# taha-kms/CLASSMATE-RAG

Measured on AMD Instinct MI355X. Metric: hybrid queries/sec + recall@10 vs reference, 10M×768 chunks, 1/2/4/8 GPU, higher is better.
Workload: dtype fp32-accurate E5 (K10 f16x3 MFMA) + int8/f16/f64 dense + f64 BM25

## Files before the change

classmate-rag_amd/classmate_hip/_lib.py:

```python
from __future__ import annotations

import ctypes as C
import os
from pathlib import Path

try:
    import torch
except Exception:
    torch = None

LIB_NAME = "libclassmate_hip.so"
LIB_PATH = Path(os.environ.get("CLASSMATE_HIP_LIB", Path(__file__).with_name(LIB_NAME)))

CM_OK, CM_EINVAL, CM_ENOMEM, CM_EDEVICE, CM_EZERODIV, CM_EUNSUPPORTED = 0, -1, -2, -3, -4, -5
CM_FOP_EQ, CM_FOP_NE, CM_FOP_BITS, CM_FOP_TRUE, CM_FOP_FALSE, CM_FOP_AND, CM_FOP_OR, CM_FOP_NOT = range(1, 9)
CM_FILTER_MAX_OPS, CM_FILTER_MAX_SOURCES = 64, 16
CM_DTYPE_F32, CM_DTYPE_BF16, CM_DTYPE_F16, CM_DTYPE_I32, CM_DTYPE_I64 = 0, 1, 2, 3, 4

if not LIB_PATH.exists():
    raise ImportError(
        f"{LIB_PATH} not found: build the HIP extension first "
        f"(python -c 'import __graft_entry__ as g; g.build()' or make -C classmate-rag_amd)")

lib = C.CDLL(str(LIB_PATH), mode=C.RTLD_GLOBAL)
# ... 11 lines not shown


SIGNATURES = {
    "cm_last_error": (c_char_p,),
    "cm_version": (c_int,),
    "cm_device_count": (c_int, P(c_int)),
    "cm_stream_create_cu_masked": (c_int, c_int, P(C.c_uint32), c_int, P(c_vp)),
    "cm_stream_destroy": (c_int, c_vp),
    "cm_max_topk": (c_int,),
    "cm_dense_create": (c_int, c_int, c_i32, c_i64, P(c_vp)),
    "cm_dense_destroy": (None, c_vp),
    "cm_dense_reserve": (c_int, c_vp, c_i64),
    "cm_dense_mem_stats": (c_int, c_vp, c_vp, c_vp, c_vp),
    "cm_dense_set_growth": (c_int, c_vp, c_i32),
    "cm_dense_upsert": (c_int, c_vp, c_vp, c_vp, c_i64),
    "cm_dense_upsert_dev": (c_int, c_vp, c_vp, c_i64, c_i64, c_vp),
    "cm_dense_delete": (c_int, c_vp, c_vp, c_i64),
    "cm_dense_compact": (c_int, c_vp, c_i64, c_i32, c_vp, c_vp),
    "cm_dense_truncate": (c_int, c_vp, c_i64),
    "cm_dense_reset": (c_int, c_vp),
    "cm_dense_live_count": (c_i64, c_vp),
    "cm_dense_size": (c_i64, c_vp),
    "cm_dense_dim": (c_i32, c_vp),
    "cm_dense_search": (c_int, c_vp, c_vp, c_i32, c_i32, c_vp, c_vp, c_vp, c_vp),
    "cm_dense_search_lists": (c_int, c_vp, c_vp, c_i32, c_i32, c_vp, c_i32, c_vp, c_vp, c_vp, c_vp),
    "cm_dense_search_lists_dev": (c_int, c_vp, c_vp, c_i32, c_i32, c_vp, c_i32, c_vp, c_vp, c_vp, c_vp),
    "cm_dense_search_workspace": (c_i64, c_vp, c_i32, c_i32),
    "cm_dense_search_kind": (c_i32, c_vp, c_i32, c_i32),
    "cm_dense_set_path": (c_int, c_vp, c_i32),
    "cm_dense_workspace_fallbacks": (c_i32, c_vp, c_i32, c_i32, c_vp),
    "cm_dense_last_fallbacks": (c_i32, c_vp),
    "cm_dense_workspace_wide_reranks": (c_i32, c_vp, c_i32, c_i32, c_vp),
    "cm_dense_last_wide_reranks": (c_i32, c_vp),
    "cm_dense_timing": (c_int, c_vp, c_i32),
    "cm_dense_set_seed_event": (c_int, c_vp, c_vp),
    "cm_dense_timing_drain": (c_i32, c_vp, c_vp, c_i32),
    "cm_bm25_timing": (c_int, c_vp, c_i32),
    "cm_bm25_timing_drain": (c_i32, c_vp, c_vp, c_i32),
    "cm_dense_search_dev": (c_int, c_vp, c_vp, c_i32, c_i32, c_vp, c_vp, c_vp, c_vp, c_i64, c_vp),
    "cm_shard_merge_topk_dev": (c_int, c_vp, c_i32, c_i32, c_i32, c_i32, c_vp, c_vp, c_vp, c_vp, c_vp),
    "cm_dense_search_dev_deferred": (c_int, c_vp, c_vp, c_i32, c_i32, c_vp, c_vp, c_vp, c_vp, c_i64, c_vp),
    "cm_dense_exact_fallback_dev": (c_int, c_vp, c_vp, c_i32, c_i32, c_vp, c_vp, c_vp, c_vp, c_i64, c_vp),
    "cm_dense_export": (c_int, c_vp, c_i64, c_i64, c_vp, c_vp),
    "cm_dense_gather_dev": (c_int, c_vp, c_vp, c_i64, c_vp, c_vp),
    "cm_dense_live_bits_dev": (c_vp, c_vp),
    "cm_bm25_create": (c_int, c_int, P(c_vp)),
    "cm_bm25_destroy": (None, c_vp),
    "cm_bm25_build": (c_int, c_vp, c_vp, c_vp, c_i64, c_i32, c_vp),
    "cm_bm25_build_dev": (c_int, c_vp, c_vp, c_vp, c_i64, c_i64, c_i32, c_vp),
    "cm_bm25_append": (c_int, c_vp, c_vp, c_vp, c_i64, c_i32),
    "cm_bm25_append_dev": (c_int, c_vp, c_vp, c_vp, c_i64, c_i64, c_i32, c_vp),
    "cm_bm25_remove": (c_int, c_vp, c_vp, c_i64),
    "cm_bm25_remove_dev": (c_int, c_vp, c_vp, c_vp),
    "cm_bm25_replace": (c_int, c_vp, c_vp, c_i64, c_vp, c_vp, c_i32),
    "cm_bm25_replace_dev": (c_int, c_vp, c_vp, c_i64, c_vp, c_vp, c_i64, c_i32, c_vp),
    "cm_bm25_num_docs": (c_i64, c_vp),
    "cm_bm25_num_postings": (c_i64, c_vp),
    "cm_bm25_stats": (c_int, c_vp, P(c_i64), P(c_i64), P(c_f64), P(c_f64)),
    "cm_bm25_export": (c_int, c_vp, c_vp, c_vp, c_vp, c_vp, c_vp),
    "cm_bm25_set_head_policy": (c_int, c_vp, c_f64, c_i64),
    "cm_bm25_num_head_terms": (c_i32, c_vp),
    "cm_bm25_set_path": (c_int, c_vp, c_i32),
    "cm_bm25_workspace_rescored": (c_i32, c_vp, c_i32, c_i32, c_i32, c_vp),
    "cm_bm25_last_rescored": (c_i32, c_vp),
    "cm_bm25_term_stats": (c_int, c_vp, c_vp, c_vp),
    "cm_bm25_set_stats": (c_int, c_vp, c_vp, c_i32, c_i64, c_i64, c_f64),
# ... 87 lines not shown
```

classmate-rag_amd/classmate_hip/engine.py:

```python
from __future__ import annotations

import ctypes as C
import os
from typing import Optional, Sequence

import numpy as np

from . import _lib as L

try:
    import torch
except Exception:
    torch = None


def default_device() -> int:
    env = os.environ.get("CM_DEVICE")
    if env:
        return int(env)
    if torch is not None and torch.cuda.is_available():
        return torch.cuda.current_device()
    return 0


# ... 195 lines not shown
            raise ValueError(f"filter_of entries must be in [0, {ab.shape[0]})")
        dist = np.empty((nq, k), np.float32)
        rows = np.empty((nq, k), np.int64)
        vecs = np.empty((nq, k, self.dim), np.float32) if return_vectors else None
        if nq:
            L.check(L.fn["cm_dense_search_lists"](self._h, L.ptr(qq), nq, int(k), L.ptr(ab), int(ab.shape[0]), L.ptr(fo),
                                                  L.ptr(dist), L.ptr(rows), L.ptr(vecs)), "cm_dense_search_lists")
        return (dist, rows, vecs) if return_vectors else (dist, rows)

    def export(self, row0: int = 0, n: Optional[int] = None, with_live: bool = False):
        n = self.size - row0 if n is None else int(n)
        out = np.empty((max(n, 0), self.dim), np.float32)
        live = np.zeros(max((n + 31) // 32, 1), np.uint32) if with_live else None
        L.check(L.fn["cm_dense_export"](self._h, int(row0), n, L.ptr(out), L.ptr(live)), "cm_dense_export")
        if not with_live:
            return out
        mask = np.unpackbits(live.view(np.uint8), bitorder="little")[:n].astype(bool)
        return out, mask

    PATH_AUTO, PATH_F32, PATH_COARSE, PATH_STREAM, PATH_Q8, PATH_Q8S = 0, 1, 3, 4, 5, 6

    def set_path(self, kind: int):
        L.check(L.fn["cm_dense_set_path"](self._h, int(kind)), "cm_dense_set_path")

    def search_kind(self, nq: int, k: int) -> int:
        return int(L.fn["cm_dense_search_kind"](self._h, int(nq), int(k)))

    def last_fallbacks(self) -> int:
        return int(L.fn["cm_dense_last_fallbacks"](self._h))

    def last_wide_reranks(self) -> int:
        return int(L.fn["cm_dense_last_wide_reranks"](self._h))

    def timing(self, enable: bool = True):
        L.check(L.fn["cm_dense_timing"](self._h, int(bool(enable))), "cm_dense_timing")

    def set_seed_event(self, event=None):
        self._seed_event = event
        L.check(L.fn["cm_dense_set_seed_event"](self._h, event.cuda_event if event is not None else None),
                "cm_dense_set_seed_event")

    def timing_drain(self, cap: int = 4096) -> list:
        buf = np.zeros(cap, np.float32)
        n = int(L.fn["cm_dense_timing_drain"](self._h, L.ptr(buf), int(cap)))
        if n < 0:
            raise RuntimeError(L.last_error())
        return buf[:min(n, cap)].tolist()

    def workspace_fallbacks(self, nq: int, k: int, workspace) -> int:
        return int(L.fn["cm_dense_workspace_fallbacks"](self._h, int(nq), int(k), L.ptr(workspace)))

    def workspace_wide_reranks(self, nq: int, k: int, workspace) -> int:
        return int(L.fn["cm_dense_workspace_wide_reranks"](self._h, int(nq), int(k), L.ptr(workspace)))

    def workspace_bytes(self, nq: int, k: int) -> int:
        n = int(L.fn["cm_dense_search_workspace"](self._h, int(nq), int(k)))
        if n < 0:
            raise ValueError("bad (nq, k) for dense search")
        return n

    def search_dev(self, q, k: int, allow=None, out=None, workspace=None, defer_exact: bool = False):
        nq = q.shape[0]
        dev = q.device
        wsb = self.workspace_bytes(nq, k)
        if workspace is None:
            if self._ws is None or self._ws.numel() < wsb:
                self._ws = torch.empty(wsb, dtype=torch.uint8, device=dev)
            workspace = self._ws
        if out is None:
            out = (torch.empty((nq, k), dtype=torch.float32, device=dev),
                   torch.empty((nq, k), dtype=torch.int64, device=dev))
        name = "cm_dense_search_dev_deferred" if defer_exact else "cm_dense_search_dev"
        L.check(L.fn[name](self._h, L.ptr(q), nq, int(k), L.ptr(allow), L.ptr(out[0]), L.ptr(out[1]),
                           L.ptr(workspace), int(workspace.numel()), _stream(self.device)), name)
        return out

    def exact_fallback_dev(self, q, k: int, out, workspace=None, allow=None):
        if workspace is None:
            workspace = self._ws
        L.check(L.fn["cm_dense_exact_fallback_dev"](self._h, L.ptr(q), q.shape[0], int(k), L.ptr(allow),
                                                    L.ptr(out[0]), L.ptr(out[1]), L.ptr(workspace),
                                                    int(workspace.numel()), _stream(self.device)),
                "cm_dense_exact_fallback_dev")
        return out

    def gather_dev(self, rows, out=None):
# ... 722 lines not shown
```

classmate-rag_amd/csrc/cm_dense.hip:

```cpp
#include "cm_common.h"

#include <hipcub/hipcub.hpp>

#include <algorithm>
#include <cstdlib>
#include <cstring>
#include <memory>
#include <mutex>
#include <vector>

namespace cm {

typedef float f32x4 __attribute__((ext_vector_type(4)));

constexpr int kWaves = 8;
constexpr int kThreads = kWaves * 64;
constexpr int kRowTile = 16;
constexpr int kStepRows = kRowTile * kWaves;
constexpr int kCap = kStepRows;

struct DenseLds {
  int qfrag, invq, thr, cnt, len, list, buf, total;
};

// ... 968 lines not shown
    }
  }
}

__global__ void popcount_kernel(const uint32_t *__restrict__ bits, int64_t n_words,
                                unsigned long long *__restrict__ out) {
  int64_t i = (int64_t)blockIdx.x * blockDim.x + threadIdx.x;
  unsigned long long c = 0;
  for (; i < n_words; i += (int64_t)gridDim.x * blockDim.x) c += __popc(bits[i]);
  for (int o = 32; o > 0; o >>= 1) c += __shfl_xor(c, o);
  if ((threadIdx.x & 63) == 0 && c) atomicAdd(out, c);
}

}

using namespace cm;

struct cm_dense {
  int dev = 0;
  int dim = 0;
  int ld = 0;
  int64_t rows_alloc = 0;
  int64_t size = 0;
  float *C = nullptr;
  float *invc = nullptr;
  _Float16 *Xh = nullptr;
  int64_t xh_rows = 0;
  int8_t *Xq = nullptr;
  float2 *rmeta = nullptr;
  float *rnorm = nullptr;
  int path = 0;
  int32_t last_fallbacks = -1;
  int32_t last_wide = -1;
  KernelTimer timer;
  hipEvent_t seed_event = nullptr;
  uint32_t *live = nullptr;
  hipStream_t stream = nullptr;
  int64_t mem_cur = 0, mem_peak = 0;
  int64_t staged_growths = 0;
  int32_t grow_mode = 0;
  DevBuf staging, rows_buf, allow_buf, ws, out_buf;
  std::vector<float> host_tmp;
};

namespace {

struct DenseCfg {
  int QB, CH, KMAX, n_qgroups, n_cblocks;
  int64_t rows_per_block, rows_end;
  size_t lds;
};

int pick_chunk(int ld) {
  const int KS = ld / 16;
  if (KS % 24 == 0) return 12;
  if (KS % 16 == 0) return 8;
  return 0;
}

int g_num_cus = 0;

int num_cus(int dev) {
  if (g_num_cus == 0) {
    hipDeviceProp_t p;
    if (hipGetDeviceProperties(&p, dev) == hipSuccess) g_num_cus = p.multiProcessorCount;
    if (g_num_cus <= 0) g_num_cus = 256;
// ... 362 lines not shown
  uint32_t *fb_bound;
  int32_t *wide_ctr;
  uint32_t *wide_rows;
  uint64_t *wide_keys;
  DenseWs k1;
  size_t total;
};
CoarseWs coarse_ws_layout(const cm_dense *h, const CoarseCfg &c, int nq, int k, void *base) {
  CoarseWs w{};
  char *p = reinterpret_cast<char *>(base);
  size_t off = 0;
  const int64_t nq_pad = (int64_t)c.n_pass * c.qs;
  auto take = [&](int64_t bytes) -> char * {
    char *r = p + off;
    off += round_up(std::max<int64_t>(bytes, 1), 256);
    return r;
  };
  const int cap = c.q8 ? kQCap : kCBufCap;
  if (c.q8) {
    w.qq = reinterpret_cast<int8_t *>(take(nq_pad * h->ld));
    w.qsc = reinterpret_cast<float4 *>(take(nq_pad * 16));
  }
  w.qh = reinterpret_cast<_Float16 *>(take(nq_pad * h->ld * 2));
  w.qnorm = reinterpret_cast<float *>(take(nq_pad * 16));
  w.keys = reinterpret_cast<uint64_t *>(take((int64_t)c.n_pass * c.n_wg * c.qs * cap * 8));
  if (c.q8) w.ups = reinterpret_cast<float *>(take((int64_t)c.n_pass * c.n_wg * c.qs * cap * 4));
  w.cnt = reinterpret_cast<uint32_t *>(take((int64_t)c.n_pass * c.n_wg * c.qs * 4));
  w.mins = reinterpret_cast<float *>(take((int64_t)c.n_pass * c.n_wg_sample * c.qs * 4));
  w.seed = reinterpret_cast<float *>(take(nq_pad * 4));
  w.fb_mask = reinterpret_cast<int32_t *>(take(nq_pad * 4));
  w.fb_count = reinterpret_cast<int32_t *>(take(4));
  if (c.q8) {
    w.fb_bound = reinterpret_cast<uint32_t *>(take(nq_pad * 4));
    w.wide_ctr = reinterpret_cast<int32_t *>(take(8));
    w.wide_rows = reinterpret_cast<uint32_t *>(take((int64_t)kWideSlots * kWideCap * 4));
    w.wide_keys = reinterpret_cast<uint64_t *>(take((int64_t)kWideSlots * kWideCap * 8));
  }
  const DenseCfg kc = dense_config(h, nq, k, true);
  w.k1 = dense_ws_layout(h, kc, k, p ? p + off : nullptr);
  off += w.k1.total;
  w.total = off;
  return w;
}

int set_coarse_attrs() {
  static std::once_flag once;
  static hipError_t err = hipSuccess;
  std::call_once(once, [] {
    const std::pair<const void *, int> fs[] = {
        {reinterpret_cast<const void *>(&dense_coarse_scan_kernel<12, kK1cNql, false>), K1rLds<kK1cNql>::total},
        {reinterpret_cast<const void *>(&dense_coarse_scan_kernel<12, kK1cNql, true>), K1rLds<kK1cNql>::total},
        {reinterpret_cast<const void *>(&dense_coarse_scan_kernel<6, 0, false>), K1rLds<0>::total},
        {reinterpret_cast<const void *>(&dense_coarse_scan_kernel<6, 0, true>), K1rLds<0>::total},
        {reinterpret_cast<const void *>(&dense_rerank_kernel), kGatherCap * 12},
        {reinterpret_cast<const void *>(&dense_q8_scan_kernel<>), kQLds},
        {reinterpret_cast<const void *>(&dense_q8_scan_kernel<K1Q_LDS_SHARED>), kQLdsShared},
        {reinterpret_cast<const void *>(&dense_rerank_q8_kernel), kQRerankLds}};
    for (const auto &f : fs) {
      const hipError_t e = hipFuncSetAttribute(f.first, hipFuncAttributeMaxDynamicSharedMemorySize, f.second);
      if (e != hipSuccess) err = e;
    }
  });
  CM_HIP(err);
  return CM_OK;
}

using StreamFn = void (*)(const _Float16 *, const uint32_t *, const uint32_t *, int64_t, const _Float16 *, int,
// ... 13 lines not shown
    lds = K1rLds<kK1cNql>::total;
    return minonly ? &dense_coarse_scan_kernel<12, kK1cNql, true> : &dense_coarse_scan_kernel<12, kK1cNql, false>;
  }
  lds = K1rLds<0>::total;
  return minonly ? &dense_coarse_scan_kernel<6, 0, true> : &dense_coarse_scan_kernel<6, 0, false>;
}
using Q8Fn = void (*)(const int8_t *, const float2 *, const uint32_t *, const uint32_t *, int64_t, const int8_t *,
                      const float4 *, int, const float *, int64_t, int64_t, int, uint64_t *, float *, uint32_t *);
Q8Fn q8_kernel(bool full, size_t &lds) {
  lds = full ? kQLds : kQLdsShared;
  return full ? &dense_q8_scan_kernel<> : &dense_q8_scan_kernel<K1Q_LDS_SHARED>;
}
Q8Fn q8_stream_kernel(int nq) {
  return nq > 16 ? &dense_q8_stream_kernel<2, K1QS_RING> : &dense_q8_stream_kernel<1, K1QS_RING>;
}

int launch_exact_fallback(cm_dense *h, const float *q_dev, int nq, int k, int kind, const uint32_t *allow,
                          float *dist_dev, int64_t *row_dev, void *ws, int64_t ws_bytes, hipStream_t st);
int launch_coarse(cm_dense *h, const float *q_dev, int nq, int k, int kind, const uint32_t *allow,
                  float *dist_dev, int64_t *row_dev, void *ws, int64_t ws_bytes, hipStream_t st,
                  bool run_exact = true) {
  int rc;
  if ((rc = set_coarse_attrs())) return rc;
  const CoarseCfg c = coarse_config(h, nq, kind);
  const CoarseWs w = coarse_ws_layout(h, c, nq, k, ws);
  if ((int64_t)w.total > ws_bytes || !ws) CM_FAIL(CM_EINVAL, "dense workspace too small");
  const int64_t n_words = ceil_div(h->size, 32);
  size_t lds = 0;
  hipLaunchKernelGGL(dense_prep_planes, dim3(c.n_pass * c.qs), dim3(256), 0, st, q_dev, nq, h->dim, h->ld, w.qh,
                     w.qnorm);
  CM_HIP(hipGetLastError());
  CM_HIP(hipMemsetAsync(w.fb_count, 0, 4, st));
  if (c.q8) {
    CM_HIP(hipMemsetAsync(w.wide_ctr, 0, 8, st));
    hipLaunchKernelGGL(dense_prep_q8, dim3(c.n_pass * c.qs), dim3(256), 0, st, q_dev, nq, h->dim, h->ld, w.qq, w.qsc,
                       reinterpret_cast<const uint32_t *>(h->rnorm));
    CM_HIP(hipGetLastError());
  }
  if (c.stream) {
    hipLaunchKernelGGL(stream_kernel(h->ld, nq, true), dim3((unsigned)ceil_div(c.n_wg_sample, 4)), dim3(256), 0, st,
                       h->Xh, h->live, allow, n_words, w.qh, nq, (const float *)nullptr, c.rows_per_wg_sample,
                       c.rows_end_sample, c.n_wg_sample, c.qs, (uint64_t *)nullptr, (uint32_t *)nullptr, w.mins);
  } else {
    const CoarseFn fn = coarse_kernel(h->ld, true, lds);
    hipLaunchKernelGGL(fn, dim3((unsigned)((int64_t)c.n_pass * c.n_wg_sample)), dim3(256), lds, st, h->Xh, h->live,
                       allow, n_words, w.qh, nq, (const float *)nullptr, c.rows_per_wg_sample, c.rows_end_sample,
                       c.n_wg_sample, (uint64_t *)nullptr, (uint32_t *)nullptr, w.mins);
  }
  CM_HIP(hipGetLastError());
  hipLaunchKernelGGL(dense_seed_kernel, dim3(nq), dim3(256), 0, st, w.mins, c.n_wg_sample, c.qs, k, nq, w.qnorm,
                     h->rnorm, h->dim, w.seed, c.q8 ? 1 : 2);
  CM_HIP(hipGetLastError());
  if (kind == CM_DENSE_Q8 && h->seed_event) CM_HIP(hipEventRecord(h->seed_event, st));
  h->timer.begin(st);
  if (c.q8s) {
    hipLaunchKernelGGL(q8_stream_kernel(nq), dim3((unsigned)ceil_div(c.n_wg, 4)), dim3(256), 0, st, h->Xq, h->rmeta,
                       h->live, allow, n_words, w.qq, w.qsc, nq, (const float *)w.seed, c.rows_per_wg, c.rows_end,
                       c.n_wg, w.keys, w.ups, w.cnt);
  } else if (c.q8) {
    const Q8Fn fn = q8_kernel(run_exact || !env_knob("CM_K1Q_SHARED_LDS", true), lds);
    hipLaunchKernelGGL(fn, dim3(c.n_pass * c.n_wg), dim3(256), lds, st, h->Xq, h->rmeta, h->live, allow, n_words,
                       w.qq, w.qsc, nq, (const float *)w.seed, c.rows_per_wg, c.rows_end, c.n_wg, w.keys, w.ups, w.cnt);
  } else if (c.stream) {
    hipLaunchKernelGGL(stream_kernel(h->ld, nq, false), dim3((unsigned)ceil_div(c.n_wg, 4)), dim3(256), 0, st, h->Xh,
                       h->live, allow, n_words, w.qh, nq, (const float *)w.seed, c.rows_per_wg, c.rows_end, c.n_wg,
                       c.qs, w.keys, w.cnt, (float *)nullptr);
  } else {
    const CoarseFn fn = coarse_kernel(h->ld, false, lds);
    hipLaunchKernelGGL(fn, dim3((unsigned)((int64_t)c.n_pass * c.n_wg)), dim3(256), lds, st, h->Xh, h->live, allow,
                       n_words, w.qh, nq, (const float *)w.seed, c.rows_per_wg, c.rows_end, c.n_wg, w.keys, w.cnt,
                       (float *)nullptr);
  }
  h->timer.end(st);
  CM_HIP(hipGetLastError());
  if (c.q8) {
    hipLaunchKernelGGL(dense_rerank_q8_kernel, dim3(nq), dim3(kQRT), kQRerankLds, st, w.keys, w.ups, w.cnt, c.n_wg,
                       c.qs, k, nq, h->C, h->ld, h->dim, q_dev, w.qsc, xh_full(h) ? h->Xh : nullptr, w.qh, w.qnorm,
                       h->rnorm, dist_dev, row_dev, w.fb_mask, w.fb_count, w.fb_bound);
    CM_HIP(hipGetLastError());
    if (env_knob("CM_K1Q_WIDE", true))
      hipLaunchKernelGGL(dense_rerank_wide_kernel, dim3(nq), dim3(kWideThreads), 0, st, w.keys, w.cnt, c.n_wg, c.qs,
                         k, nq, h->C, h->ld, h->dim, q_dev, w.qsc, xh_full(h) ? h->Xh : nullptr, w.qh, w.qnorm,
                         h->rnorm, h->Xq, h->rmeta, w.qq, h->live, allow, n_words, c.rows_per_wg, c.rows_end, dist_dev,
                         row_dev, w.fb_mask, w.fb_count, w.fb_bound, w.wide_ctr, w.wide_rows, w.wide_keys);
  } else {
    hipLaunchKernelGGL(dense_rerank_kernel, dim3(nq), dim3(256), kGatherCap * 12, st, w.keys, w.cnt, c.n_wg, c.qs, k,
                       nq, h->C, h->ld, h->dim, q_dev, w.qnorm, h->rnorm, dist_dev, row_dev, w.fb_mask, w.fb_count);
  }
  CM_HIP(hipGetLastError());
  return run_exact ? launch_exact_fallback(h, q_dev, nq, k, kind, allow, dist_dev, row_dev, ws, ws_bytes, st) : CM_OK;
}

int launch_exact_fallback(cm_dense *h, const float *q_dev, int nq, int k, int kind, const uint32_t *allow,
                          float *dist_dev, int64_t *row_dev, void *ws, int64_t ws_bytes, hipStream_t st) {
  const CoarseCfg c = coarse_config(h, nq, kind);
  const CoarseWs w = coarse_ws_layout(h, c, nq, k, ws);
  if ((int64_t)w.total > ws_bytes || !ws) CM_FAIL(CM_EINVAL, "dense workspace too small");
  const DenseCfg kc = dense_config(h, nq, k, true);
  if (kc.lds > 163840) CM_FAIL(CM_EUNSUPPORTED, "dim/k too large for the LDS-resident query tile");
  hipLaunchKernelGGL(dense_prep_queries, dim3(kc.n_qgroups * kc.QB), dim3(256), 0, st, q_dev, nq, h->dim, h->ld,
                     w.k1.qp, w.k1.invq);
  CM_HIP(hipGetLastError());
  int rc;
  if ((rc = launch_dense(kc, h, allow, w.k1.qp, w.k1.invq, nq, k, w.fb_mask, w.fb_count, w.k1.cand, st))) return rc;
  hipLaunchKernelGGL(dense_merge_kernel, dim3(nq), dim3(256), 0, st, w.k1.cand, kc.n_cblocks, kc.QB, k, nq,
                     (const int32_t *)w.fb_mask, dist_dev, row_dev);
  CM_HIP(hipGetLastError());
  return CM_OK;
}

int dense_search_full(cm_dense *h, const float *q, int nq, int k, const uint32_t *allow_bits, float *out_dist,
// ... 21 lines not shown
  std::vector<uint64_t> top((size_t)kk);
  std::vector<float> qpad((size_t)h->ld, 0.f);
  for (int i = 0; i < nq; ++i) {
    double qn = 0.0;
    for (int c = 0; c < h->dim; ++c) {
      qpad[c] = q[(int64_t)i * h->dim + c];
      qn += (double)qpad[c] * qpad[c];
    }
    CM_HIP(hipMemcpyAsync(qp, qpad.data(), (size_t)h->ld * 4, hipMemcpyHostToDevice, h->stream));
    hipLaunchKernelGGL(dense_all_keys_kernel, dim3((unsigned)ceil_div(n, 16)), dim3(256), 0, h->stream, h->C, h->ld,
                       h->live, allow_dev, h->size, qp, std::sqrt(qn), keys);
    CM_HIP(hipGetLastError());
    CM_HIP(hipcub::DeviceRadixSort::SortKeys(base, tmp_bytes, keys, sorted, (int)n, 0, 64, h->stream));
    CM_HIP(hipMemcpyAsync(top.data(), sorted, (size_t)kk * 8, hipMemcpyDeviceToHost, h->stream));
    CM_HIP(hipStreamSynchronize(h->stream));
    for (int j = 0; j < k; ++j) {
      const uint64_t key = j < kk ? top[j] : kEmptyKey;
      out_dist[(int64_t)i * k + j] = key == kEmptyKey ? 0.f : f32_unorder((uint32_t)(key >> 32));
      out_row[(int64_t)i * k + j] = key == kEmptyKey ? -1 : (int64_t)(uint32_t)key;
    }
  }
  if (out_vec) {
    const size_t nr = (size_t)nq * k;
    if ((rc = h->rows_buf.ensure(nr * 8)) || (rc = h->out_buf.ensure(nr * h->dim * 4))) return rc;
    CM_HIP(hipMemcpyAsync(h->rows_buf.ptr, out_row, nr * 8, hipMemcpyHostToDevice, h->stream));
    hipLaunchKernelGGL(dense_gather_kernel, dim3((unsigned)nr), dim3(256), 0, h->stream, h->C, h->ld, h->dim,
                       h->rows_buf.as<int64_t>(), (int64_t)nr, h->size, h->out_buf.as<float>());
    CM_HIP(hipGetLastError());
    CM_HIP(hipMemcpyAsync(out_vec, h->out_buf.ptr, nr * h->dim * 4, hipMemcpyDeviceToHost, h->stream));
    CM_HIP(hipStreamSynchronize(h->stream));
  }
  h->last_fallbacks = 0;
  h->last_wide = 0;
  return CM_OK;
}

}

extern "C" {

int cm_max_topk(void) { return kMaxTopK; }

int cm_dense_create(int device, int32_t dim, int64_t capacity, cm_dense **out) {
  if (!out) CM_FAIL(CM_EINVAL, "out is NULL");
  *out = nullptr;
  if (dim <= 0 || dim > 2048) CM_FAIL(CM_EINVAL, "dim must be in [1, 2048]");
  if (capacity < 0) CM_FAIL(CM_EINVAL, "capacity must be >= 0");
  DeviceGuard dg(device);
  if (!dg.ok) CM_FAIL(CM_EDEVICE, "cannot select device " + std::to_string(device));
  cm_dense *h = new cm_dense();
  h->dev = device;
  h->dim = dim;
  int ld = (int)round_up(dim, 128);
  while (!pick_chunk(ld)) ld += 128;
  h->ld = ld;
  if (hipStreamCreateWithFlags(&h->stream, hipStreamDefault) != hipSuccess) {
    delete h;
    CM_FAIL(CM_EDEVICE, "hipStreamCreate failed");
  }
  if (hipMalloc(&h->rnorm, 16) != hipSuccess || hipMemset(h->rnorm, 0, 16) != hipSuccess) {
    cm_dense_destroy(h);
    CM_FAIL(CM_ENOMEM, "dense: out of device memory");
  }
  int rc = dense_grow(h, std::max<int64_t>(capacity, kStepRows));
  if (rc) {
    cm_dense_destroy(h);
// ... 168 lines not shown
int cm_dense_set_path(cm_dense *h, int32_t kind) {
  if (!h) CM_FAIL(CM_EINVAL, "null handle");
  if (kind < 0 || kind > CM_DENSE_Q8S) CM_FAIL(CM_EINVAL, "unknown dense path");
  h->path = kind;
  return CM_OK;
}

int32_t cm_dense_workspace_fallbacks(cm_dense *h, int32_t nq, int32_t k, const void *workspace_dev) {
  if (!h || !workspace_dev || nq <= 0 || k <= 0 || k > kMaxTopK) return -1;
  const int kind = dense_kind(h, nq, k);
  if (kind == CM_DENSE_F32) return 0;
  DeviceGuard dg(h->dev);
  const CoarseWs w = coarse_ws_layout(h, coarse_config(h, nq, kind), nq, k,
                                      const_cast<void *>(workspace_dev));
  int32_t c = -1;
  if (hipMemcpy(&c, w.fb_count, 4, hipMemcpyDeviceToHost) != hipSuccess) return -1;
  return c;
}

int32_t cm_dense_last_fallbacks(cm_dense *h) { return h ? h->last_fallbacks : -1; }

int32_t cm_dense_workspace_wide_reranks(cm_dense *h, int32_t nq, int32_t k, const void *workspace_dev) {
  if (!h || !workspace_dev || nq <= 0 || k <= 0 || k > kMaxTopK) return -1;
  const int kind = dense_kind(h, nq, k);
  if (kind != CM_DENSE_Q8 && kind != CM_DENSE_Q8S) return 0;
  DeviceGuard dg(h->dev);
  const CoarseWs w = coarse_ws_layout(h, coarse_config(h, nq, kind), nq, k, const_cast<void *>(workspace_dev));
  int32_t c[2] = {-1, -1};
  if (hipMemcpy(c, w.wide_ctr, 8, hipMemcpyDeviceToHost) != hipSuccess) return -1;
  return c[1];
}

int32_t cm_dense_last_wide_reranks(cm_dense *h) { return h ? h->last_wide : -1; }

int cm_dense_set_seed_event(cm_dense *h, void *event) {
  if (!h) CM_FAIL(CM_EINVAL, "null handle");
  h->seed_event = (hipEvent_t)event;
  return CM_OK;
}

int cm_dense_timing(cm_dense *h, int32_t enable) {
  if (!h) CM_FAIL(CM_EINVAL, "null handle");
  DeviceGuard dg(h->dev);
  h->timer.on = enable != 0;
  h->timer.used = 0;
  return CM_OK;
}

int32_t cm_dense_timing_drain(cm_dense *h, float *ms_out, int32_t cap) {
  if (!h) CM_FAIL(CM_EINVAL, "null handle");
  DeviceGuard dg(h->dev);
  const int n = h->timer.drain(ms_out, cap);
  if (n < 0) CM_FAIL(CM_EDEVICE, "event query failed");
  return n;
}

int32_t cm_dense_search_kind(cm_dense *h, int32_t nq, int32_t k) {
  if (!h || nq <= 0 || k <= 0 || k > kMaxTopK) return -1;
  return dense_kind(h, nq, k);
}

int cm_dense_search_dev(cm_dense *h, const float *q_dev, int32_t nq, int32_t k, const uint32_t *allow_dev,
                        float *dist_dev, int64_t *row_dev, void *workspace_dev, int64_t workspace_bytes,
                        void *stream) {
  if (!h) CM_FAIL(CM_EINVAL, "null handle");
  if (nq <= 0) return CM_OK;
// ... 91 lines not shown
  DeviceGuard dg(h->dev);
  if (k > kMaxTopK) return dense_search_full(h, q, nq, k, allow_bits, out_dist, out_row, out_vec);
  const int64_t wsb = cm_dense_search_workspace(h, nq, k);
  int rc;
  if ((rc = h->ws.ensure((size_t)wsb))) return rc;
  const size_t qbytes = (size_t)nq * h->dim * 4;
  const size_t obytes = (size_t)nq * k * (4 + 8);
  const size_t vbytes = out_vec ? (size_t)nq * k * h->dim * 4 : 0;
  if ((rc = h->staging.ensure(qbytes))) return rc;
  if ((rc = h->out_buf.ensure(round_up(obytes, 256) + vbytes))) return rc;
  const uint32_t *allow_dev = nullptr;
  if (allow_bits) {
    const int64_t nw = ceil_div(h->size, 32);
    if ((rc = h->allow_buf.ensure((size_t)std::max<int64_t>(nw, 1) * 4))) return rc;
    CM_HIP(hipMemcpyAsync(h->allow_buf.ptr, allow_bits, (size_t)nw * 4, hipMemcpyDefault, h->stream));
    allow_dev = h->allow_buf.as<uint32_t>();
  }
  CM_HIP(hipMemcpyAsync(h->staging.ptr, q, qbytes, hipMemcpyHostToDevice, h->stream));
  float *d_dist = h->out_buf.as<float>();
  int64_t *d_row = reinterpret_cast<int64_t *>(h->out_buf.as<char>() + round_up((int64_t)nq * k * 4, 8));
  rc = cm_dense_search_dev(h, h->staging.as<float>(), nq, k, allow_dev, d_dist, d_row, h->ws.ptr, wsb, h->stream);
  if (rc) return rc;
  float *d_vec = nullptr;
  if (out_vec) {
    d_vec = reinterpret_cast<float *>(h->out_buf.as<char>() + round_up(obytes, 256));
    rc = cm_dense_gather_dev(h, d_row, (int64_t)nq * k, d_vec, h->stream);
    if (rc) return rc;
  }
  CM_HIP(hipMemcpyAsync(out_dist, d_dist, (size_t)nq * k * 4, hipMemcpyDeviceToHost, h->stream));
  CM_HIP(hipMemcpyAsync(out_row, d_row, (size_t)nq * k * 8, hipMemcpyDeviceToHost, h->stream));
  if (out_vec) CM_HIP(hipMemcpyAsync(out_vec, d_vec, vbytes, hipMemcpyDeviceToHost, h->stream));
  h->last_fallbacks = 0;
  h->last_wide = 0;
  const int kind = dense_kind(h, nq, k);
  if (kind != CM_DENSE_F32) {
    const CoarseWs w = coarse_ws_layout(h, coarse_config(h, nq, kind), nq, k, h->ws.ptr);
    CM_HIP(hipMemcpyAsync(&h->last_fallbacks, w.fb_count, 4, hipMemcpyDeviceToHost, h->stream));
    if (w.wide_ctr) CM_HIP(hipMemcpyAsync(&h->last_wide, w.wide_ctr + 1, 4, hipMemcpyDeviceToHost, h->stream));
  }
  CM_HIP(hipStreamSynchronize(h->stream));
  return CM_OK;
}

}

#include "cm_dense_compact.inc"
#include "cm_dense_lists.inc"
```

classmate-rag_amd/csrc/cm_dense_q8.inc:

```

#ifndef K1Q_RING
#define K1Q_RING 12
#endif
#ifndef K1Q_DBG
#define K1Q_DBG 0
#endif
constexpr int kQDbg = K1Q_DBG;
constexpr int kQRing = K1Q_RING;
constexpr int kQCap = 128;
#ifndef K1Q_RR
#define K1Q_RR 4096
#endif
#ifndef K1Q_RT
#define K1Q_RT 1024
#endif
constexpr int kQBand = K1Q_RR;
constexpr int kQBand2 = K1Q_RR / 2;
constexpr int kQRT = K1Q_RT, kQRW = K1Q_RT / 64;
constexpr int kQSel = 256;
constexpr int kQMeta = 4;
#ifndef K1Q_LDS
#define K1Q_LDS (160 * 1024)
#endif
#ifndef K1Q_LDS_SHARED
// ... 660 lines not shown
      uint32_t incl = sum;
#pragma unroll
      for (int o = 1; o < 64; o <<= 1) {
        const uint32_t v = __shfl_up(incl, o);
        if (l >= o) incl += v;
      }
      const uint32_t rem = s_rem, excl = incl - sum;
      if (excl <= rem && rem < incl) {
        uint32_t r = rem - excl, b = 4u * l;
        if (r >= h0) {
          r -= h0;
          ++b;
          if (r >= h1) {
            r -= h1;
            ++b;
            if (r >= h2) {
              r -= h2;
              ++b;
            }
          }
        }
        s_prefix = prefix | (b << shift);
        s_rem = r;
      }
    }
    __syncthreads();
  }
  return s_prefix;
}

constexpr int kQGather = K1Q_RR;
constexpr int kQRows = 8;
constexpr int kQRerankLds = kQGather * 12;
__global__ void __launch_bounds__(kQRT) dense_rerank_q8_kernel(
    const uint64_t *__restrict__ keys, const float *__restrict__ ups, const uint32_t *__restrict__ cnts, int n_wg,
    int qs, int k, int nq, const float *__restrict__ C, int ld, int dim, const float *__restrict__ q,
    const float4 *__restrict__ qsc, const _Float16 *__restrict__ Xh, const _Float16 *__restrict__ Qh,
    const float *__restrict__ qnorm, const float *__restrict__ row_norms, float *__restrict__ out_dist,
    int64_t *__restrict__ out_row, int32_t *__restrict__ fb_mask, int32_t *__restrict__ fb_count,
    uint32_t *__restrict__ fb_bound) {
  const int qi = blockIdx.x;
  if (qi >= nq) return;
  const int tid = threadIdx.x, lane = tid & 63, wave = tid >> 6;
  const int qp = qi / qs, ql = qi - qp * qs;
  extern __shared__ __attribute__((aligned(16))) unsigned char dyn[];
  uint64_t *g_key = reinterpret_cast<uint64_t *>(dyn);
  uint32_t *g_up = reinterpret_cast<uint32_t *>(dyn + kQGather * 8);
  __shared__ uint32_t s_off[2049];
  __shared__ uint32_t hist[256];
  __shared__ float s_q[768];
  __shared__ int s_flag, s_total, s_band;
  __shared__ uint64_t s_sel[kQSel];
  __shared__ int s_nsel;
  static_assert(kQBand * 4 <= kQGather * 4 && kQBand * 4 <= kQGather * 4 && kQBand2 * 8 <= kQGather * 4, "K1q re-rank LDS");
  uint32_t *s_rows = g_up;
  uint64_t *s_ex = g_key;
  if (tid == 0) {
    s_flag = 0;
    s_band = 0;
    s_nsel = 0;
  }
  __syncthreads();
  if (wave == 0) {
    uint32_t run = 0;
    for (int b0 = 0; b0 < n_wg; b0 += 64) {
      const int b = b0 + lane;
      uint32_t c = b < n_wg ? cnts[((int64_t)qp * n_wg + b) * qs + ql] : 0u;
      if (c > (uint32_t)kQCap) {
        s_flag = 1;
        c = kQCap;
      }
      uint32_t incl = c;
      for (int o = 1; o < 64; o <<= 1) {
// ... 12 lines not shown
  const int total = s_total;
  auto slot_of = [&](int jj) -> int64_t {
    int lo = 0, hi = n_wg - 1;
    while (lo < hi) {
      const int mid = (lo + hi + 1) >> 1;
      if (s_off[mid] <= (uint32_t)jj) lo = mid;
      else hi = mid - 1;
    }
    return (((int64_t)qp * n_wg + lo) * qs + ql) * kQCap + (jj - s_off[lo]);
  };
  const bool gathered = total <= kQGather;
  if (gathered) {
#pragma unroll 4
    for (int jj = tid; jj < total; jj += kQRT) {
      const int64_t sl = slot_of(jj);
      g_key[jj] = keys[sl];
      g_up[jj] = f32_order(ups[sl]);
    }
  }
  for (int i = tid; i < 768; i += kQRT) s_q[i] = i < dim ? q[(int64_t)qi * dim + i] : 0.f;
  __syncthreads();
  auto key_at = [&](int jj) -> uint64_t { return gathered ? g_key[jj] : keys[slot_of(jj)]; };
  auto up_at = [&](int jj) -> uint32_t { return gathered ? g_up[jj] : f32_order(ups[slot_of(jj)]); };
  uint32_t tkey = 0xffffffffu;
  if (total >= k) tkey = block_select_fn(up_at, total, k - 1, hist);
  if (s_flag) {
    if (tid == 0) {
      fb_mask[qi] = 2;
      fb_bound[qi] = tkey;
      atomicAdd(fb_count, 1);
    }
    return;
  }
  for (int jj = tid; jj < total; jj += kQRT) {
    const uint64_t key = key_at(jj);
    if (tkey == 0xffffffffu || (uint32_t)(key >> 32) <= tkey) {
      const int p = atomicAdd(&s_band, 1);
      if (p < kQBand) s_rows[p] = (uint32_t)key;
    }
  }
  __syncthreads();
  const int band = s_band;
  if (band > kQBand) {
    if (tid == 0) {
      fb_mask[qi] = 2;
      fb_bound[qi] = tkey;
      atomicAdd(fb_count, 1);
    }
    return;
  }
  if (tid == 0) {
    fb_mask[qi] = 0;
    fb_bound[qi] = 0u;
  }
  const uint32_t *band_rows = s_rows;
  int band2 = band;
  if (Xh != nullptr) {
  float *s_dh = reinterpret_cast<float *>(dyn);
  uint32_t *s_rows2 = reinterpret_cast<uint32_t *>(dyn + kQGather * 4);
  const float Eh = coarse_err(qnorm, qi, row_norms, dim);
  {
    typedef _Float16 h2 __attribute__((ext_vector_type(2)));
    const int hl = lane & 31, hh = lane >> 5;
    f16x8 qv[3];
    int kof[3];
#pragma unroll
    for (int u = 0; u < 3; ++u) {
      const int pc = hl + 32 * u;
      kof[u] = 64 * (pc >> 3) + 32 * ((pc >> 2) & 1) + 8 * (pc & 3);
      qv[u] = *reinterpret_cast<const f16x8 *>(Qh + (int64_t)qi * ld + kof[u]);
    }
    constexpr int RP = 4;
    for (int c0 = wave * 2 * RP; c0 < band; c0 += kQRW * 2 * RP) {
      f16x8 xv[RP][3];
#pragma unroll
      for (int rp = 0; rp < RP; ++rp) {
        const int c = min(c0 + 2 * rp + hh, band - 1);
        const int64_t row = s_rows[c];
        const int64_t tile = row >> 6;
        const int rr = (int)(row & 63), rt = rr >> 4, jj = rr & 15;
// ... 4 lines not shown
              Xh + ((((tile * (ld >> 6) + cch) * 8 + rt * 2 + sb) << 9) + ((jj * 4 + gg) << 3)));
        }
      }
#pragma unroll
      for (int rp = 0; rp < RP; ++rp) {
        float acc = 0.f;
#pragma unroll
        for (int u = 0; u < 3; ++u)
#pragma unroll
          for (int e = 0; e < 8; e += 2)
            acc = __builtin_amdgcn_fdot2(h2{xv[rp][u][e], xv[rp][u][e + 1]}, h2{qv[u][e], qv[u][e + 1]}, acc, false);
#pragma unroll
        for (int o = 16; o > 0; o >>= 1) acc += __shfl_xor(acc, o);
        const int c = c0 + 2 * rp + hh;
        if (hl == 0 && c < band) s_dh[c] = 1.0f - acc;
      }
    }
  }
  __syncthreads();
  {
    const uint32_t kth_h = band >= k ? block_select_fn([&](int i) { return f32_order(s_dh[i] + Eh); }, band, k - 1, hist)
                                     : 0xffffffffu;
    if (tid == 0) s_band = 0;
    __syncthreads();
    for (int c = tid; c < band; c += kQRT)
      if (kth_h == 0xffffffffu || f32_order(s_dh[c] - Eh) <= kth_h) s_rows2[atomicAdd(&s_band, 1)] = s_rows[c];
    __syncthreads();
  }
  band2 = s_band;
  band_rows = s_rows2;
  if (band2 > kQBand2) {
    if (tid == 0) {
      fb_mask[qi] = 2;
      fb_bound[qi] = tkey;
      atomicAdd(fb_count, 1);
    }
    return;
  }
  }
  const double qnrm = (double)qsc[qi].w;
  constexpr int M = 12;
  for (int c0 = wave * kQRows; c0 < band2; c0 += kQRW * kQRows) {
    float x[kQRows][M];
    uint32_t rows[kQRows];
#pragma unroll
    for (int r = 0; r < kQRows; ++r) {
      const int c = min(c0 + r, band2 - 1);
      rows[r] = band_rows[c];
      const float *cr = C + (int64_t)rows[r] * ld + lane;
#pragma unroll
      for (int m = 0; m < M; ++m) x[r][m] = cr[64 * m];
    }
    double dq[kQRows], dc[kQRows];
#pragma unroll
    for (int r = 0; r < kQRows; ++r) {
      dq[r] = 0.0;
      dc[r] = 0.0;
#pragma unroll
      for (int m = 0; m < M; ++m) {
        const double xv = (double)x[r][m];
        dq[r] += xv * (double)s_q[lane + 64 * m];
        dc[r] += xv * xv;
      }
    }
    for (int o = 32; o > 0; o >>= 1) {
#pragma unroll
      for (int r = 0; r < kQRows; ++r) {
        dq[r] += __shfl_xor(dq[r], o);
        dc[r] += __shfl_xor(dc[r], o);
      }
    }
    if (lane == 0) {
#pragma unroll
      for (int r = 0; r < kQRows; ++r)
        if (c0 + r < band2) {
          const float dist = (float)(1.0 - dq[r] / ((sqrt(dc[r]) + 1e-30) * (qnrm + 1e-30)));
          s_ex[c0 + r] = ((uint64_t)f32_order(dist) << 32) | rows[r];
        }
    }
  }
  __syncthreads();
  const uint32_t thi = band2 > k ? block_select_fn([&](int i) { return (uint32_t)(s_ex[i] >> 32); }, band2, k - 1, hist)
                                : 0xffffffffu;
  for (int c = tid; c < band2; c += kQRT) {
    const uint64_t key = s_ex[c];
    if ((uint32_t)(key >> 32) <= thi) {
      const int p = atomicAdd(&s_nsel, 1);
      if (p < kQSel) s_sel[p] = key;
    }
  }
  __syncthreads();
  const int nsel = s_nsel;
  const uint64_t *cand = nsel <= kQSel ? s_sel : s_ex;
  const int ncand = nsel <= kQSel ? nsel : band2;
  for (int c = tid; c < ncand; c += kQRT) {
    const uint64_t key = cand[c];
    int rank = 0;
    for (int i = 0; i < ncand; ++i) rank += cand[i] < key ? 1 : 0;
    if (rank < k) {
      out_dist[(int64_t)qi * k + rank] = f32_unorder((uint32_t)(key >> 32));
      out_row[(int64_t)qi * k + rank] = (int64_t)(uint32_t)key;
    }
  }
  for (int i = band2 + tid; i < k; i += kQRT) {
    out_dist[(int64_t)qi * k + i] = 0.f;
    out_row[(int64_t)qi * k + i] = -1;
  }
}

constexpr int kWideSlots = 16;
constexpr int kWideCap = 1 << 16;
constexpr int kWideThreads = 1024;
constexpr int kWideOvf = 64;
// ... 235 lines not shown
```

include/classmate_hip.h:

```cpp
#ifndef CLASSMATE_HIP_H
#define CLASSMATE_HIP_H

#include <stddef.h>
#include <stdint.h>

#ifdef __cplusplus
extern "C" {
#endif

#define CM_OK 0
#define CM_EINVAL (-1)
#define CM_ENOMEM (-2)
#define CM_EDEVICE (-3)
#define CM_EZERODIV (-4)
#define CM_EUNSUPPORTED (-5)

#define CM_DTYPE_F32 0
#define CM_DTYPE_BF16 1
#define CM_DTYPE_F16 2
#define CM_DTYPE_I32 3
#define CM_DTYPE_I64 4

const char *cm_last_error(void);
int cm_version(void);
// ... 9 lines not shown
int cm_dense_reserve(cm_dense *h, int64_t capacity);
int cm_dense_mem_stats(cm_dense *h, int64_t *cur_bytes, int64_t *peak_bytes, int64_t *staged_growths);
int cm_dense_set_growth(cm_dense *h, int32_t mode);
int cm_dense_upsert(cm_dense *h, const float *vecs, const int64_t *rows, int64_t n);
int cm_dense_upsert_dev(cm_dense *h, const float *vecs_dev, int64_t row0, int64_t n, void *stream);
int cm_dense_delete(cm_dense *h, const int64_t *rows, int64_t n);
int cm_dense_compact(cm_dense *h, int64_t expect_live, int32_t shrink, int64_t *old_rows_out, int64_t *new_size);
int cm_dense_truncate(cm_dense *h, int64_t new_size);
int cm_dense_reset(cm_dense *h);
int64_t cm_dense_live_count(cm_dense *h);
int64_t cm_dense_size(cm_dense *h);
int32_t cm_dense_dim(cm_dense *h);
int cm_dense_search(cm_dense *h, const float *q, int32_t nq, int32_t k, const uint32_t *allow_bits,
                    float *out_dist, int64_t *out_row, float *out_vec);
int cm_dense_search_lists(cm_dense *h, const float *q, int32_t nq, int32_t k, const uint32_t *allow_bits,
                          int32_t n_filters, const int32_t *filter_of, float *out_dist, int64_t *out_row,
                          float *out_vec);
int cm_dense_search_lists_dev(cm_dense *h, const float *q_dev, int32_t nq, int32_t k, const uint32_t *allow_bits,
                              int32_t n_filters, const int32_t *filter_of, float *dist_dev, int64_t *row_dev,
                              void *stream);
int64_t cm_dense_search_workspace(cm_dense *h, int32_t nq, int32_t k);
#define CM_DENSE_F32 1
#define CM_DENSE_F16X3 2
#define CM_DENSE_COARSE 3
#define CM_DENSE_STREAM 4
#define CM_DENSE_Q8 5
#define CM_DENSE_Q8S 6
int32_t cm_dense_search_kind(cm_dense *h, int32_t nq, int32_t k);
int cm_dense_set_path(cm_dense *h, int32_t kind);
int32_t cm_dense_workspace_fallbacks(cm_dense *h, int32_t nq, int32_t k, const void *workspace_dev);
int32_t cm_dense_last_fallbacks(cm_dense *h);
int32_t cm_dense_workspace_wide_reranks(cm_dense *h, int32_t nq, int32_t k, const void *workspace_dev);
int32_t cm_dense_last_wide_reranks(cm_dense *h);
int cm_dense_timing(cm_dense *h, int32_t enable);
int cm_dense_set_seed_event(cm_dense *h, void *event);
int32_t cm_dense_timing_drain(cm_dense *h, float *ms_out, int32_t cap);
int cm_dense_search_dev(cm_dense *h, const float *q_dev, int32_t nq, int32_t k, const uint32_t *allow_dev,
                        float *dist_dev, int64_t *row_dev, void *workspace_dev, int64_t workspace_bytes,
                        void *stream);
int cm_dense_search_dev_deferred(cm_dense *h, const float *q_dev, int32_t nq, int32_t k, const uint32_t *allow_dev,
                                 float *dist_dev, int64_t *row_dev, void *workspace_dev, int64_t workspace_bytes,
                                 void *stream);
int cm_dense_exact_fallback_dev(cm_dense *h, const float *q_dev, int32_t nq, int32_t k, const uint32_t *allow_dev,
                                float *dist_dev, int64_t *row_dev, void *workspace_dev, int64_t workspace_bytes,
                                void *stream);
int cm_dense_export(cm_dense *h, int64_t row0, int64_t n, float *out, uint32_t *live_out);
int cm_dense_gather_dev(cm_dense *h, const int64_t *rows_dev, int64_t n, float *out_dev, void *stream);
const uint32_t *cm_dense_live_bits_dev(cm_dense *h);

typedef struct cm_bm25 cm_bm25;

int cm_bm25_create(int device, cm_bm25 **out);
void cm_bm25_destroy(cm_bm25 *h);
int cm_bm25_build(cm_bm25 *h, const int32_t *term_ids, const int64_t *doc_off, int64_t ndocs, int32_t vocab,
                  const uint8_t *live);
int cm_bm25_build_dev(cm_bm25 *h, const int32_t *term_ids_dev, const int64_t *doc_off_dev, int64_t ndocs,
                      int64_t ntokens, int32_t vocab, void *stream);
int cm_bm25_append(cm_bm25 *h, const int32_t *term_ids, const int64_t *doc_off, int64_t n_new, int32_t vocab);
int cm_bm25_append_dev(cm_bm25 *h, const int32_t *term_ids_dev, const int64_t *doc_off_dev, int64_t n_new,
                       int64_t ntokens, int32_t vocab, void *stream);
int cm_bm25_remove(cm_bm25 *h, const int64_t *rows, int64_t n_rows);
int cm_bm25_remove_dev(cm_bm25 *h, const uint32_t *remove_bits_dev, void *stream);
int cm_bm25_replace(cm_bm25 *h, const int64_t *rows, int64_t n_rows, const int32_t *term_ids, const int64_t *doc_off,
                    int32_t vocab);
int cm_bm25_replace_dev(cm_bm25 *h, const int64_t *rows_dev, int64_t n_rows, const int32_t *term_ids_dev,
                        const int64_t *doc_off_dev, int64_t ntokens, int32_t vocab, void *stream);
// ... 132 lines not shown
```

Before: 34640.

## Add pilot exact-rerank to tighten q8 band bound before full rerank

In the q8 rerank kernel, candidates whose upper bound is at or below the top-k threshold are first scored exactly in fp64 as a pilot set. Their k-th exact distance, plus a small pad, gives a tighter bound that shrinks the band of rows needing exact reranking and may avoid overflow fallbacks. The exact-scoring loop is factored into a templated helper, and a device counter of band rows is added for diagnostics. It adds extra block syncs and a selection pass per query, and correctness depends on the padded pilot bound staying conservative.

After: 35110 (median of 6 runs). 1.01x the previous value.

```diff
diff --git a/classmate-rag_amd/classmate_hip/_lib.py b/classmate-rag_amd/classmate_hip/_lib.py
--- a/classmate-rag_amd/classmate_hip/_lib.py
+++ b/classmate-rag_amd/classmate_hip/_lib.py
@@ -67,6 +67,8 @@
     "cm_dense_last_fallbacks": (c_i32, c_vp),
     "cm_dense_workspace_wide_reranks": (c_i32, c_vp, c_i32, c_i32, c_vp),
     "cm_dense_last_wide_reranks": (c_i32, c_vp),
+    "cm_dense_workspace_band_rows": (c_i64, c_vp, c_i32, c_i32, c_vp),
+    "cm_dense_last_band_rows": (c_i64, c_vp),
     "cm_dense_timing": (c_int, c_vp, c_i32),
     "cm_dense_set_seed_event": (c_int, c_vp, c_vp),
     "cm_dense_timing_drain": (c_i32, c_vp, c_vp, c_i32),
diff --git a/classmate-rag_amd/classmate_hip/engine.py b/classmate-rag_amd/classmate_hip/engine.py
--- a/classmate-rag_amd/classmate_hip/engine.py
+++ b/classmate-rag_amd/classmate_hip/engine.py
@@ -251,6 +251,9 @@
     def last_wide_reranks(self) -> int:
         return int(L.fn["cm_dense_last_wide_reranks"](self._h))
 
+    def last_band_rows(self) -> int:
+        return int(L.fn["cm_dense_last_band_rows"](self._h))
+
     def timing(self, enable: bool = True):
         L.check(L.fn["cm_dense_timing"](self._h, int(bool(enable))), "cm_dense_timing")
 
@@ -271,6 +274,9 @@
 
     def workspace_wide_reranks(self, nq: int, k: int, workspace) -> int:
         return int(L.fn["cm_dense_workspace_wide_reranks"](self._h, int(nq), int(k), L.ptr(workspace)))
+
+    def workspace_band_rows(self, nq: int, k: int, workspace) -> int:
+        return int(L.fn["cm_dense_workspace_band_rows"](self._h, int(nq), int(k), L.ptr(workspace)))
 
     def workspace_bytes(self, nq: int, k: int) -> int:
         n = int(L.fn["cm_dense_search_workspace"](self._h, int(nq), int(k)))
diff --git a/classmate-rag_amd/csrc/cm_dense.hip b/classmate-rag_amd/csrc/cm_dense.hip
--- a/classmate-rag_amd/csrc/cm_dense.hip
+++ b/classmate-rag_amd/csrc/cm_dense.hip
@@ -1024,6 +1024,7 @@
   int path = 0;
   int32_t last_fallbacks = -1;
   int32_t last_wide = -1;
+  int64_t last_band = -1;
   KernelTimer timer;
   hipEvent_t seed_event = nullptr;
   uint32_t *live = nullptr;
@@ -1452,7 +1453,7 @@
   w.fb_count = reinterpret_cast<int32_t *>(take(4));
   if (c.q8) {
     w.fb_bound = reinterpret_cast<uint32_t *>(take(nq_pad * 4));
-    w.wide_ctr = reinterpret_cast<int32_t *>(take(8));
+    w.wide_ctr = reinterpret_cast<int32_t *>(take(16));
     w.wide_rows = reinterpret_cast<uint32_t *>(take((int64_t)kWideSlots * kWideCap * 4));
     w.wide_keys = reinterpret_cast<uint64_t *>(take((int64_t)kWideSlots * kWideCap * 8));
   }
@@ -1532,7 +1533,7 @@
   CM_HIP(hipGetLastError());
   CM_HIP(hipMemsetAsync(w.fb_count, 0, 4, st));
   if (c.q8) {
-    CM_HIP(hipMemsetAsync(w.wide_ctr, 0, 8, st));
+    CM_HIP(hipMemsetAsync(w.wide_ctr, 0, 16, st));
     hipLaunchKernelGGL(dense_prep_q8, dim3(c.n_pass * c.qs), dim3(256), 0, st, q_dev, nq, h->dim, h->ld, w.qq, w.qsc,
                        reinterpret_cast<const uint32_t *>(h->rnorm));
     CM_HIP(hipGetLastError());
@@ -1574,9 +1575,11 @@
   h->timer.end(st);
   CM_HIP(hipGetLastError());
   if (c.q8) {
+    const bool pilot = env_knob("CM_K1Q_PILOT", true);
     hipLaunchKernelGGL(dense_rerank_q8_kernel, dim3(nq), dim3(kQRT), kQRerankLds, st, w.keys, w.ups, w.cnt, c.n_wg,
                        c.qs, k, nq, h->C, h->ld, h->dim, q_dev, w.qsc, xh_full(h) ? h->Xh : nullptr, w.qh, w.qnorm,
-                       h->rnorm, dist_dev, row_dev, w.fb_mask, w.fb_count, w.fb_bound);
+                       h->rnorm, dist_dev, row_dev, w.fb_mask, w.fb_count, w.fb_bound,
+                       pilot ? 1 : 0, reinterpret_cast<unsigned long long *>(w.wide_ctr + 2));
     CM_HIP(hipGetLastError());
     if (env_knob("CM_K1Q_WIDE", true))
       hipLaunchKernelGGL(dense_rerank_wide_kernel, dim3(nq), dim3(kWideThreads), 0, st, w.keys, w.cnt, c.n_wg, c.qs,
@@ -1664,6 +1667,7 @@
   }
   h->last_fallbacks = 0;
   h->last_wide = 0;
+  h->last_band = 0;
   return CM_OK;
 }
 
@@ -1898,6 +1902,19 @@
 }
 
 int32_t cm_dense_last_wide_reranks(cm_dense *h) { return h ? h->last_wide : -1; }
+
+int64_t cm_dense_workspace_band_rows(cm_dense *h, int32_t nq, int32_t k, const void *workspace_dev) {
+  if (!h || !workspace_dev || nq <= 0 || k <= 0 || k > kMaxTopK) return -1;
+  const int kind = dense_kind(h, nq, k);
+  if (kind != CM_DENSE_Q8 && kind != CM_DENSE_Q8S) return 0;
+  DeviceGuard dg(h->dev);
+  const CoarseWs w = coarse_ws_layout(h, coarse_config(h, nq, kind), nq, k, const_cast<void *>(workspace_dev));
+  int64_t c = -1;
+  if (hipMemcpy(&c, w.wide_ctr + 2, 8, hipMemcpyDeviceToHost) != hipSuccess) return -1;
+  return c;
+}
+
+int64_t cm_dense_last_band_rows(cm_dense *h) { return h ? h->last_band : -1; }
 
 int cm_dense_set_seed_event(cm_dense *h, void *event) {
   if (!h) CM_FAIL(CM_EINVAL, "null handle");
@@ -2055,11 +2072,15 @@
   if (out_vec) CM_HIP(hipMemcpyAsync(out_vec, d_vec, vbytes, hipMemcpyDeviceToHost, h->stream));
   h->last_fallbacks = 0;
   h->last_wide = 0;
+  h->last_band = 0;
   const int kind = dense_kind(h, nq, k);
   if (kind != CM_DENSE_F32) {
     const CoarseWs w = coarse_ws_layout(h, coarse_config(h, nq, kind), nq, k, h->ws.ptr);
     CM_HIP(hipMemcpyAsync(&h->last_fallbacks, w.fb_count, 4, hipMemcpyDeviceToHost, h->stream));
-    if (w.wide_ctr) CM_HIP(hipMemcpyAsync(&h->last_wide, w.wide_ctr + 1, 4, hipMemcpyDeviceToHost, h->stream));
+    if (w.wide_ctr) {
+      CM_HIP(hipMemcpyAsync(&h->last_wide, w.wide_ctr + 1, 4, hipMemcpyDeviceToHost, h->stream));
+      CM_HIP(hipMemcpyAsync(&h->last_band, w.wide_ctr + 2, 8, hipMemcpyDeviceToHost, h->stream));
+    }
   }
   CM_HIP(hipStreamSynchronize(h->stream));
   return CM_OK;
diff --git a/classmate-rag_amd/csrc/cm_dense_q8.inc b/classmate-rag_amd/csrc/cm_dense_q8.inc
--- a/classmate-rag_amd/csrc/cm_dense_q8.inc
+++ b/classmate-rag_amd/csrc/cm_dense_q8.inc
@@ -716,13 +716,59 @@
 constexpr int kQGather = K1Q_RR;
 constexpr int kQRows = 8;
 constexpr int kQRerankLds = kQGather * 12;
+constexpr uint32_t kQPilotPad = 4;
+constexpr int kQPilotRows = 2;
+constexpr uint64_t kQTaken = ~0ull;
+
+template <int NR, typename R>
+__device__ __forceinline__ void q8_exact_rows(const R *src, int n, int c0, int stride, const float *__restrict__ C,
+                                              int ld, const float *s_q, double qnrm, int lane, uint64_t *out) {
+  constexpr int M = 12;
+  float x[NR][M];
+  uint32_t rows[NR];
+#pragma unroll
+  for (int r = 0; r < NR; ++r) {
+    rows[r] = (uint32_t)src[min(c0 + r * stride, n - 1)];
+    const float *cr = C + (int64_t)rows[r] * ld + lane;
+#pragma unroll
+    for (int m = 0; m < M; ++m) x[r][m] = cr[64 * m];
+  }
+  double dq[NR], dc[NR];
+#pragma unroll
+  for (int r = 0; r < NR; ++r) {
+    dq[r] = 0.0;
+    dc[r] = 0.0;
+#pragma unroll
+    for (int m = 0; m < M; ++m) {
+      const double xv = (double)x[r][m];
+      dq[r] += xv * (double)s_q[lane + 64 * m];
+      dc[r] += xv * xv;
+    }
+  }
+  for (int o = 32; o > 0; o >>= 1) {
+#pragma unroll
+    for (int r = 0; r < NR; ++r) {
+      dq[r] += __shfl_xor(dq[r], o);
+      dc[r] += __shfl_xor(dc[r], o);
+    }
+  }
+  if (lane == 0) {
+#pragma unroll
+    for (int r = 0; r < NR; ++r)
+      if (c0 + r * stride < n) {
+        const float dist = (float)(1.0 - dq[r] / ((sqrt(dc[r]) + 1e-30) * (qnrm + 1e-30)));
+        out[c0 + r * stride] = ((uint64_t)f32_order(dist) << 32) | rows[r];
+      }
+  }
+}
+
 __global__ void __launch_bounds__(kQRT) dense_rerank_q8_kernel(
     const uint64_t *__restrict__ keys, const float *__restrict__ ups, const uint32_t *__restrict__ cnts, int n_wg,
     int qs, int k, int nq, const float *__restrict__ C, int ld, int dim, const float *__restrict__ q,
     const float4 *__restrict__ qsc, const _Float16 *__restrict__ Xh, const _Float16 *__restrict__ Qh,
     const float *__restrict__ qnorm, const float *__restrict__ row_norms, float *__restrict__ out_dist,
     int64_t *__restrict__ out_row, int32_t *__restrict__ fb_mask, int32_t *__restrict__ fb_count,
-    uint32_t *__restrict__ fb_bound) {
+    uint32_t *__restrict__ fb_bound, int pilot, unsigned long long *__restrict__ band_ctr) {
   const int qi = blockIdx.x;
   if (qi >= nq) return;
   const int tid = threadIdx.x, lane = tid & 63, wave = tid >> 6;
@@ -801,20 +847,54 @@
     }
     return;
   }
+  const double qnrm = (double)qsc[qi].w;
+  uint32_t bound = tkey;
+  int npilot = 0;
+  if (pilot && Xh == nullptr && total >= k) {
+    for (int jj = tid; jj < total; jj += kQRT) {
+      if (up_at(jj) <= tkey) {
+        const int p = atomicAdd(&s_nsel, 1);
+        if (p < kQSel) s_sel[p] = (uint64_t)jj;
+      }
+    }
+    __syncthreads();
+    npilot = s_nsel;
+    __syncthreads();
+    if (tid == 0) s_nsel = 0;
+    if (npilot <= kQSel) {
+      static_assert(kQSel <= kQRT, "one thread per pilot row");
+      if (tid < npilot) {
+        const int jj = (int)s_sel[tid];
+        s_sel[tid] = (uint32_t)key_at(jj);
+        if (gathered) g_key[jj] = kQTaken;
+      }
+      __syncthreads();
+      for (int c0 = wave; c0 < npilot; c0 += kQRW * kQPilotRows)
+        q8_exact_rows<kQPilotRows>(s_sel, npilot, c0, kQRW, C, ld, s_q, qnrm, lane, s_sel);
+      __syncthreads();
+      const uint32_t pkey = block_select_fn([&](int i) { return (uint32_t)(s_sel[i] >> 32); }, npilot, k - 1, hist);
+      bound = min(tkey, pkey <= 0xffffffffu - kQPilotPad ? pkey + kQPilotPad : 0xffffffffu);
+    } else {
+      npilot = 0;
+    }
+  }
+  const bool pilot_by_up = npilot > 0 && !gathered;
   for (int jj = tid; jj < total; jj += kQRT) {
     const uint64_t key = key_at(jj);
-    if (tkey == 0xffffffffu || (uint32_t)(key >> 32) <= tkey) {
+    if (key == kQTaken || (pilot_by_up && up_at(jj) <= tkey)) continue;
+    if (bound == 0xffffffffu || (uint32_t)(key >> 32) <= bound) {
       const int p = atomicAdd(&s_band, 1);
       if (p < kQBand) s_rows[p] = (uint32_t)key;
     }
   }
   __syncthreads();
   const int band = s_band;
-  if (band > kQBand) {
+  if (band + npilot > kQBand) {
     if (tid == 0) {
       fb_mask[qi] = 2;
-      fb_bound[qi] = tkey;
+      fb_bound[qi] = bound;
       atomicAdd(fb_count, 1);
+      if (npilot) atomicAdd(band_ctr, (unsigned long long)npilot);
     }
     return;
   }
@@ -885,53 +965,17 @@
   if (band2 > kQBand2) {
     if (tid == 0) {
       fb_mask[qi] = 2;
-      fb_bound[qi] = tkey;
+      fb_bound[qi] = bound;
       atomicAdd(fb_count, 1);
     }
     return;
   }
   }
-  const double qnrm = (double)qsc[qi].w;
-  constexpr int M = 12;
-  for (int c0 = wave * kQRows; c0 < band2; c0 += kQRW * kQRows) {
-    float x[kQRows][M];
-    uint32_t rows[kQRows];
-#pragma unroll
-    for (int r = 0; r < kQRows; ++r) {
-      const int c = min(c0 + r, band2 - 1);
-      rows[r] = band_rows[c];
-      const float *cr = C + (int64_t)rows[r] * ld + lane;
-#pragma unroll
-      for (int m = 0; m < M; ++m) x[r][m] = cr[64 * m];
-    }
-    double dq[kQRows], dc[kQRows];
-#pragma unroll
-    for (int r = 0; r < kQRows; ++r) {
-      dq[r] = 0.0;
-      dc[r] = 0.0;
-#pragma unroll
-      for (int m = 0; m < M; ++m) {
-        const double xv = (double)x[r][m];
-        dq[r] += xv * (double)s_q[lane + 64 * m];
-        dc[r] += xv * xv;
-      }
-    }
-    for (int o = 32; o > 0; o >>= 1) {
-#pragma unroll
-      for (int r = 0; r < kQRows; ++r) {
-        dq[r] += __shfl_xor(dq[r], o);
-        dc[r] += __shfl_xor(dc[r], o);
-      }
-    }
-    if (lane == 0) {
-#pragma unroll
-      for (int r = 0; r < kQRows; ++r)
-        if (c0 + r < band2) {
-          const float dist = (float)(1.0 - dq[r] / ((sqrt(dc[r]) + 1e-30) * (qnrm + 1e-30)));
-          s_ex[c0 + r] = ((uint64_t)f32_order(dist) << 32) | rows[r];
-        }
-    }
-  }
+  if (tid == 0) atomicAdd(band_ctr, (unsigned long long)(band2 + npilot));
+  for (int c0 = wave * kQRows; c0 < band2; c0 += kQRW * kQRows)
+    q8_exact_rows<kQRows>(band_rows, band2, c0, 1, C, ld, s_q, qnrm, lane, s_ex);
+  if (tid < npilot) s_ex[band2 + tid] = s_sel[tid];
+  band2 += npilot;
   __syncthreads();
   const uint32_t thi = band2 > k ? block_select_fn([&](int i) { return (uint32_t)(s_ex[i] >> 32); }, band2, k - 1, hist)
                                 : 0xffffffffu;
diff --git a/include/classmate_hip.h b/include/classmate_hip.h
--- a/include/classmate_hip.h
+++ b/include/classmate_hip.h
@@ -65,6 +65,8 @@
 int32_t cm_dense_last_fallbacks(cm_dense *h);
 int32_t cm_dense_workspace_wide_reranks(cm_dense *h, int32_t nq, int32_t k, const void *workspace_dev);
 int32_t cm_dense_last_wide_reranks(cm_dense *h);
+int64_t cm_dense_workspace_band_rows(cm_dense *h, int32_t nq, int32_t k, const void *workspace_dev);
+int64_t cm_dense_last_band_rows(cm_dense *h);
 int cm_dense_timing(cm_dense *h, int32_t enable);
 int cm_dense_set_seed_event(cm_dense *h, void *event);
 int32_t cm_dense_timing_drain(cm_dense *h, float *ms_out, int32_t cap);
```
